# spawner1145/vae-tagger

Measured on AMD Instinct MI355X. Metric: images/sec encode+tag, 1024^2 bf16, higher is better.
Workload: dtype bf16

## Files before the change

### include/vae_tagger_hip.h

```cpp
#ifndef VAE_TAGGER_HIP_H
#define VAE_TAGGER_HIP_H

#include <stddef.h>
#include <stdint.h>

#ifdef __cplusplus
extern "C" {
#endif

typedef struct vt_context vt_context;

enum { VT_OK = 0, VT_ERR_INVALID = 1, VT_ERR_HIP = 2, VT_ERR_STATE = 3, VT_ERR_MISSING_WEIGHT = 4,
       VT_ERR_WORKSPACE = 5 };
enum { VT_F32 = 0, VT_BF16 = 1, VT_F16 = 2, VT_U8 = 3  };

const char* vt_version(void);
int vt_create(int device, vt_context** out);
void vt_destroy(vt_context* ctx);
const char* vt_last_error(const vt_context* ctx);

int vt_encoder_configure(vt_context* ctx, int in_channels, int latent_channels, const int* block_out_channels,
                         int n_blocks, int layers_per_block, int norm_num_groups, float scaling_factor,
                         int has_scaling_factor, float shift_factor, int has_shift_factor);
int vt_set_weight(vt_context* ctx, const char* name, const void* host_data, int dtype, const int64_t* shape,
// ... 107 lines not shown
                    size_t workspace_bytes, void* stream);
int vt_head_forward_backward(vt_context* ctx, void* state, size_t state_bytes, const float* features, const void* labels, int labels_dtype,
                             int B, int loss_kind, double focal_alpha, double focal_gamma, const float* class_weights, double loss_scale,
                             int train, const float* dropout_p , unsigned long long seed, unsigned long long step,
                             float* logits_out, unsigned char* masks_out, void* workspace, size_t workspace_bytes, void* stream);
int vt_head_clip(vt_context* ctx, void* state, size_t state_bytes, float max_norm, void* stream);
int vt_head_step(vt_context* ctx, void* state, size_t state_bytes, double lr, double beta1, double beta2, double eps, double weight_decay,
                 long long t, void* stream);
int vt_head_commit(vt_context* ctx, const void* state, size_t state_bytes, void* stream);
int vt_head_read(vt_context* ctx, const void* state, size_t state_bytes, int kind, const char* name, void* out, size_t out_bytes, void* stream);
int vt_head_write(vt_context* ctx, void* state, size_t state_bytes, int kind, const char* name, const void* src, size_t src_bytes,
                  void* stream);

int vt_set_flag(vt_context* ctx, int flag, int value);

int vt_debug_trace(vt_context* ctx, int enable, unsigned long long* sums_out, int max_sums, int* n_out);
int vt_profile_num_configs(void);
int vt_profile_begin(vt_context* ctx);
int vt_profile_end(vt_context* ctx, int max_cfg, long long* launches, double* total_ms, double* total_flops,
                   const char** kernel_names);

int vt_op_conv2d(vt_context* ctx, const void* x_bf16_nhwc, const void* w_bf16_ohwi, const float* bias,
                 const float* residual_f32, float* out_f32, void* out_bf16, int B, int Hin, int Win, int Cin,
                 int Cout, int ksize, int stride, int pad_lo, int pad_hi, void* stream);
int vt_op_norm_silu_conv3x3(vt_context* ctx, const void* x_nhwc, int x_dtype, const float* scale_shift,
                            const void* w_bf16_ohwi, const float* bias, const float* residual_f32, float* out_f32,
                            void* out_bf16, int B, int H, int W, int Cin, int Cout, void* stream);
size_t vt_op_conv2d_gn_workspace_bytes(int B, int Hout, int Wout, int Cout);
int vt_op_conv2d_gn(vt_context* ctx, const void* x_bf16_nhwc, const void* w_bf16_ohwi, const float* bias,
                    const float* residual_f32, float* out_f32, void* out_bf16, int B, int Hin, int Win, int Cin,
// ... 25 lines not shown
```

### vae_tagger_amd/_lib.py

```python
import ctypes
import os
import threading

_HERE = os.path.dirname(os.path.abspath(__file__))
LIB_PATH = os.environ.get("VAE_TAGGER_HIP_LIB") or os.path.join(_HERE, "csrc", "libvae_tagger_hip.so")

VT_F32, VT_BF16, VT_F16, VT_U8 = 0, 1, 2, 3
VT_STATUS_NONFINITE, VT_STATUS_FP8_SATURATED = 1, 2
ENCODE_MOMENTS, ENCODE_MODE, ENCODE_MODE_SCALED = 0, 1, 2
HEAD_PARAM, HEAD_GRAD, HEAD_ADAM_M, HEAD_ADAM_V, HEAD_LOSS_RING, HEAD_NORM = range(6)
HEAD_LOSS_KINDS = {"bce": 0, "focal": 1, "class_balanced": 2}
HEAD_RING = 256
VT_SAMPLE_GT, VT_SAMPLE_GE = 0, 1

_c = ctypes
_vp, _i, _f, _sz, _ll = _c.c_void_p, _c.c_int, _c.c_float, _c.c_size_t, _c.c_longlong


class ResizeItem(_c.Structure):
    _fields_ = [("src_hwc", _vp), ("src_h", _i), ("src_w", _i), ("crop_left", _i), ("crop_top", _i), ("crop_w", _i), ("crop_h", _i)]


class EvalSource(_c.Structure):
    _fields_ = [("state", _vp), ("state_bytes", _sz), ("capacity", _ll), ("n_seen", _ll)]
# ... 56 lines not shown
    "vt_decoder_feature_dim": (_i, [_vp]),
    "vt_decode_features": (_i, [_vp, _vp, _i, _i, _i, _vp, _vp, _sz, _vp]),
    "vt_head_state_bytes": (_sz, [_vp]),
    "vt_head_workspace_bytes": (_sz, [_vp, _i]),
    "vt_head_init": (_i, [_vp, _vp, _sz, _vp]),
    "vt_head_forward": (_i, [_vp, _vp, _sz, _vp, _i, _vp, _vp, _sz, _vp]),
    "vt_head_forward_backward": (_i, [_vp, _vp, _sz, _vp, _vp, _i, _i, _i, _c.c_double, _c.c_double, _vp, _c.c_double, _i,
                                      _c.POINTER(_f), _c.c_ulonglong, _c.c_ulonglong, _vp, _vp, _vp, _sz, _vp]),
    "vt_head_clip": (_i, [_vp, _vp, _sz, _f, _vp]),
    "vt_head_step": (_i, [_vp, _vp, _sz, _c.c_double, _c.c_double, _c.c_double, _c.c_double, _c.c_double, _ll, _vp]),
    "vt_head_commit": (_i, [_vp, _vp, _sz, _vp]),
    "vt_head_read": (_i, [_vp, _vp, _sz, _i, _c.c_char_p, _vp, _sz, _vp]),
    "vt_head_write": (_i, [_vp, _vp, _sz, _i, _c.c_char_p, _vp, _sz, _vp]),
    "vt_encoder_flops": (_c.c_double, [_vp, _i, _i]),
    "vt_set_flag": (_i, [_vp, _i, _i]),
    "vt_debug_trace": (_i, [_vp, _i, _c.POINTER(_c.c_ulonglong), _i, _c.POINTER(_i)]),
    "vt_profile_num_configs": (_i, []),
    "vt_profile_begin": (_i, [_vp]),
    "vt_profile_end": (_i, [_vp, _i, _c.POINTER(_ll), _c.POINTER(_c.c_double), _c.POINTER(_c.c_double), _c.POINTER(_c.c_char_p)]),
    "vt_op_conv2d": (_i, [_vp, _vp, _vp, _vp, _vp, _vp, _vp, _i, _i, _i, _i, _i, _i, _i, _i, _i, _vp]),
    "vt_op_norm_silu_conv3x3": (_i, [_vp, _vp, _i, _vp, _vp, _vp, _vp, _vp, _vp, _i, _i, _i, _i, _i, _vp]),
    "vt_op_conv2d_gn_workspace_bytes": (_sz, [_i, _i, _i, _i]),
    "vt_op_conv2d_gn": (_i, [_vp, _vp, _vp, _vp, _vp, _vp, _vp, _i, _i, _i, _i, _i, _i, _i, _i, _i, _i, _f, _vp, _vp, _vp, _vp, _vp]),
    "vt_op_conv3x3_fp8_workspace_bytes": (_sz, [_i, _i, _i, _i, _i]),
    "vt_op_conv3x3_fp8": (_i, [_vp, _vp, _vp, _vp, _vp, _vp, _i, _i, _i, _i, _i, _i, _vp, _vp]),
    "vt_op_gemm_nt": (_i, [_vp, _vp, _vp, _vp, _vp, _vp, _i, _i, _i, _i, _i, _i, _i, _ll, _ll, _ll, _f, _i, _vp]),
    "vt_op_conv_in": (_i, [_vp, _vp, _vp, _vp, _vp, _vp, _i, _i, _i, _i, _vp, _vp]),
    "vt_op_groupnorm_workspace_bytes": (_sz, [_i, _i, _i]),
    "vt_op_groupnorm": (_i, [_vp, _vp, _i, _i, _i, _i, _i, _f, _vp, _vp, _i, _vp, _vp, _vp]),
    "vt_op_softmax_rows": (_i, [_vp, _vp, _vp, _i, _i, _i, _i, _vp]),
# ... 81 lines not shown
```

### vae_tagger_amd/csrc/attention.hip

```cpp
#include <math.h>

#include "vt_context.h"

namespace vt {
namespace {

size_t attn_pitch(int S) {
    const size_t ld = (size_t)(S + 7) / 8 * 8;
    return (ld * 2) % 2048 == 0 ? ld + 2048 + 64 : ld;
}
size_t attn_pitch8(int S) {
    const size_t ld = (size_t)(S + 15) / 16 * 16;
    return ld % 2048 == 0 ? ld + 2048 + 64 : ld;
}
constexpr float FP8_QK_SCALE = 8.0f;
constexpr float FP8_P_SCALE_LOG2 = 8.0f;
constexpr float FP8_P_SCALE_SAMPLED_LOG2 = 5.0f;
int attn_group(int B, int S) {
    const size_t ld = attn_pitch(S);
    const size_t per_img = (size_t)S * ld * 4;
    size_t g = ((size_t)37 << 28) / (per_img ? per_img : 1);
    if (g < 1) g = 1;
    if (g > (size_t)B) g = (size_t)B;
    const size_t ngroups = ((size_t)B + g - 1) / g;
// ... 46 lines not shown
bool attn_proj_is_fp8(const vt_context* c, const AttnW& w, int S, int C) { return attn_is_fp8(c, S, C) && c->proj_fp8 && w.wqk8 && w.wv8; }

namespace {

int split_for(long long qblocks, int nkt) { int n = 1; while (n < nkt && qblocks * n < 512) n *= 2; return n < nkt ? n : nkt; }
int sweep_nsplit(int qblocks, int ktiles, int min_tiles) { int n = qblocks > 128 ? 1 : qblocks > 64 ? 2 : 4; while (n > 1 && ktiles / n < min_tiles) n >>= 1; return n; }

struct AttnRun {
    vt_context* c; const AttnW& w; const AttnScratch& sc; int B, S, C; hipStream_t s;
    int ld;
    int lp;
    int ld8, kext8;
    bool f8, p8;
    float scale;
    int mode;
    bool qk_kernel() const { return c->attn_qk_kernel && vt_attn_qk_supported(S, C); }
    ConvGemmArgs gemm() const {
        ConvGemmArgs a{};
        a.zeros = c->zeros; a.ksize = 1; a.stride = 1; a.pad = 0; a.Hin = a.Hout = 1; a.alpha = 1.f;
        return a;
    }
};

int attn_project(const AttnRun& r, const bf16_t* x16, bool x_e4m3) {
    vt_context* c = r.c; const AttnW& w = r.w; const AttnScratch& sc = r.sc; hipStream_t s = r.s;
    const int B = r.B, S = r.S, C = r.C, lp = r.lp;
    if (r.p8) {
        const unsigned char* x8 = (const unsigned char*)x16;
        if (!x_e4m3) {
            std::vector<float> id((size_t)B * C * 2);
// ... 16 lines not shown
        pv.out8 = sc.vt8; pv.ldo = r.ld8; pv.o_bs = (long long)C * r.ld8; pv.kext = r.kext8;
        pv.qbias = w.bv; pv.alpha = w.sv / FP8_ACT_SCALE; pv.oscale = FP8_QK_SCALE; pv.status = c->status;
        pv.C = C; pv.batch = B; pv.zeros = c->zeros;
        pv.nsplit = split_for((long long)B * ((C + 255) / 256), (S + 127) / 128);
        VTCK(profiled(c, s, VT_PROF_PROJ_FP8, 2.0 * B * (double)S * 2 * C * C, "attn qk proj fp8", [&] { return vt_launch_proj_fp8(pq, s); }));
        return profiled(c, s, VT_PROF_PROJ_FP8, 2.0 * B * (double)S * C * C, "attn v proj fp8", [&] { return vt_launch_proj_fp8(pv, s); });
    }
    if (c->attn_proj_kernel && r.qk_kernel() && (lp % 8) == 0) {
        AttnQkArgs pq{};
        pq.mode = 4; pq.q = x16; pq.ldq = C; pq.qk_bs = (long long)S * C; pq.S = S; pq.C = C;
        pq.k = w.wqk; pq.ldk = C; pq.k_bs = 0; pq.nk = 2 * C; pq.kbias = w.bqk;
        pq.P = sc.qk; pq.ldp = 2 * C; pq.p_bs = (long long)S * 2 * C; pq.alpha = 1.f; pq.batch = B; pq.zeros = c->zeros; pq.row_bs = S;
        pq.nsplit = split_for((long long)B * ((S + 255) / 256), (2 * C + 63) / 64);
        AttnQkArgs pv{};
        pv.mode = 4; pv.q = w.wv; pv.ldq = C; pv.qk_bs = 0; pv.S = C; pv.C = C; pv.qbias = w.bv;
        pv.k = x16; pv.ldk = C; pv.k_bs = (long long)S * C; pv.nk = S;
        pv.P = sc.vt; pv.ldp = lp; pv.p_bs = (long long)C * lp; pv.alpha = 1.f; pv.batch = B; pv.zeros = c->zeros; pv.row_bs = C;
        pv.nsplit = split_for((long long)B * ((C + 255) / 256), (S + 63) / 64);
        VTCK(profiled(c, s, VT_PROF_PROJ_BF16, 2.0 * B * (double)S * 2 * C * C, "attn qk proj", [&] { return vt_launch_attn_qk(pq, s); }));
        return profiled(c, s, VT_PROF_PROJ_BF16, 2.0 * B * (double)S * C * C, "attn v proj", [&] { return vt_launch_attn_qk(pv, s); });
    }
    ConvGemmArgs a = r.gemm();
    a.X = x16; a.W = w.wqk; a.bias = w.bqk; a.bias_mode = 1; a.out_bf16 = sc.qk;
    a.Win = a.Wout = S; a.Cin = C; a.Cout = 2 * C; a.Wrows = 2 * C; a.ldx = C; a.ldw = C; a.ldo = 2 * C;
    a.x_bs = (long long)S * C; a.w_bs = 0; a.o_bs = (long long)S * 2 * C; a.batch = B;
    VTCK(launch_gemm(c, a, s, "attn qk proj"));
    a.X = w.wv; a.W = x16; a.bias = w.bv; a.bias_mode = 2; a.out_bf16 = sc.vt;
    a.Win = a.Wout = C; a.Cin = C; a.Cout = r.ld; a.Wrows = S; a.ldx = C; a.ldw = C; a.ldo = lp;
    a.x_bs = 0; a.w_bs = (long long)S * C; a.o_bs = (long long)C * lp; a.batch = B;
    return launch_gemm(c, a, s, "attn v proj");
}

int attn_group_fp8(const AttnRun& r, int b0, int nb) {
    vt_context* c = r.c; const AttnScratch& sc = r.sc; hipStream_t s = r.s;
    const int S = r.S, C = r.C;
// ... 77 lines not shown
    HIPCK(c, vt_launch_attn_qk(k, s), "attn row max");
    k.mode = 2; k.P = sc.probs; k.ldp = lp; k.p_bs = (long long)S * lp; k.rowin = shift; k.rowout = rinv; k.gate = nullptr;
    const bool frag_pv = c->attn_pv_kernel && vt_attn_pv_supported(S, C);
    if (frag_pv) {
        if ((size_t)4 * nb * S > sc.group * attn_slots_bound(S) * (size_t)S) return c->fail(VT_ERR_WORKSPACE, "attention: segment sums exceed the scratch");
        k.p_frag = 1; k.p_bs = vt_attn_pt_elems(S);
        k.rowout = sc.part; k.split_stride = (long long)nb * S;
        k.nsplit = sweep_nsplit(nb * ((S + 255) / 256), (S + 63) / 64, 8);
    }
    VTCK(profiled(c, s, VT_PROF_ATTN_QK, 2.0 * nb * (double)S * S * C, "attn exp scores", [&] { return vt_launch_attn_qk(k, s); }));
    if (!frag_pv) return attn_pv_gemm(r, a, b0, rinv);
    AttnPvArgs v{};
    v.Pt = sc.probs; v.pt_bs = vt_attn_pt_elems(S); v.vt = sc.vt + (long long)b0 * C * lp; v.ldv = lp; v.vt_bs = (long long)C * lp;
    v.rsum = sc.part; v.split_stride = (long long)nb * S; v.row_bs = S; v.o = sc.o + (long long)b0 * S * C; v.ldo = C; v.o_bs = (long long)S * C;
    v.S = S; v.C = C; v.batch = nb; v.zeros = c->zeros;
    return profiled(c, s, VT_PROF_ATTN_PV, 2.0 * nb * (double)S * S * C, "attn pv", [&] { return vt_launch_attn_pv(v, s); });
}

int attn_out_proj(const AttnRun& r, const void* res, void* out, GnState* gn, int groups, int rdt) {
    vt_context* c = r.c; const AttnW& w = r.w; const AttnScratch& sc = r.sc; hipStream_t s = r.s;
    const int B = r.B, S = r.S, C = r.C;
    if (gn) gn->parts = 0;
    if (c->attn_proj_kernel && r.qk_kernel() && (C % 16) == 0) {
        AttnQkArgs po{};
        po.mode = 5; po.q = sc.o; po.ldq = C; po.qk_bs = (long long)S * C; po.S = S; po.C = C;
        po.k = w.wo; po.ldk = C; po.k_bs = 0; po.nk = C; po.kbias = w.bo;
        po.ldp = C; po.p_bs = (long long)S * C; po.alpha = 1.f; po.batch = B; po.zeros = c->zeros; po.row_bs = S;
        if (rdt == 1) { po.res_f32 = (const float*)res; po.out_f32 = (float*)out; } else { po.res_f16 = (const f16_t*)res; po.out_f16 = (f16_t*)out; }
        if (gn && c->fuse_gn_stats && C / groups == 16) { po.gn_partial = gn->partial; po.gn_parts = vt_attn_linear_parts(S); gn->parts = po.gn_parts; }
        po.nsplit = split_for((long long)B * ((S + 255) / 256), (C + 63) / 64);
// ... 5 lines not shown
    a.Win = a.Wout = S; a.Cin = C; a.Cout = C; a.Wrows = C; a.ldx = C; a.ldw = C; a.ldo = C; a.ldr = C;
    a.x_bs = (long long)S * C; a.w_bs = 0; a.o_bs = a.x_bs; a.r_bs = a.x_bs; a.batch = B;
    const int cpg = C / groups;
    if (gn && c->fuse_gn_stats && (cpg == 4 || cpg == 8 || cpg == 16) && C > 32 && (C % (C <= 128 ? 128 : 256)) == 0) {
        a.short_tiles = c->gemm_short;
        a.gn_partial = gn->partial; a.gn_cpg = cpg; gn->parts = vt_conv_gemm_ptiles_of(a);
    }
    return launch_gemm(c, a, s, "attn out proj");
}

}

int run_attention(vt_context* c, const AttnW& w, const bf16_t* x16, const void* res, void* out, int B, int S,
                  const AttnScratch& sc, hipStream_t s, GnState* gn, int groups, int rdt, bool x_e4m3) {
    const int C = w.c;
    const AttnRun r{c, w, sc, B, S, C, s, (S + 7) / 8 * 8, (int)attn_pitch(S), (int)attn_pitch8(S), (S + 15) / 16 * 16,
                    attn_is_fp8(c, S, C), attn_proj_is_fp8(c, w, S, C), 1.0f / sqrtf((float)C), c->attn_mode};
    if (x_e4m3 && !r.p8) return c->fail(VT_ERR_STATE, "internal: e4m3 tokens for a bf16 projection");
    VTCK(attn_project(r, x16, x_e4m3));
    if (r.f8) {
        HIPCK(c, hipMemsetAsync(sc.flags, 0, (size_t)((B + sc.group - 1) / sc.group) * 4, s), "attn flags");
        if (!r.p8) HIPCK(c, vt_launch_attn_row_norms_fp8(sc.qk, (long long)B * S, C, FP8_QK_SCALE, sc.qk8, sc.qn, sc.kn, sc.sd, c->status, s), "attn q|k -> e4m3");
    } else if (r.mode == 0) {
        HIPCK(c, hipMemsetAsync(sc.flags, 0, (size_t)((B + sc.group - 1) / sc.group) * 4, s), "attn flags");
        HIPCK(c, vt_launch_attn_row_norms(sc.qk, (long long)B * S, C, sc.qn, sc.kn, sc.sd, s), "attn row norms");
        HIPCK(c, vt_launch_attn_shift(sc.qn, sc.kn, sc.sd, B, S, r.scale, 120.f, sc.shift, sc.flags, sc.group, s), "attn shift");
    }
    if (r.f8 && !r.p8) HIPCK(c, vt_launch_attn_vt_to_fp8(sc.vt, (long long)C * r.lp, r.lp, sc.vt8, (long long)C * r.ld8, r.ld8, S, r.kext8, C, B, FP8_QK_SCALE, c->status, s), "attn v^T fp8");
    for (int b0 = 0; b0 < B; b0 += sc.group) VTCK(attn_group_scores_pv(r, b0, B - b0 < sc.group ? B - b0 : sc.group));
    return attn_out_proj(r, res, out, gn, groups, rdt);
}

}

using namespace vt;

extern "C" {

size_t vt_op_attention_workspace_bytes(int B, int S, int C) {
    if (B <= 0 || S <= 0 || C <= 0) return 0;
    return attn_scratch_bytes(B, S, C) + ALIGN;
}

int vt_op_attention(vt_context* c, const void* x16, const float* res, float* out, int B, int S, int C, void* ws, void* stream) {
// ... 10 lines not shown
```

### vae_tagger_amd/csrc/attn_pv.hip

```cpp
#include <hip/hip_runtime.h>

#include "vt_common.h"
#include "vt_kernels.h"

namespace {

constexpr int QB = 256;
constexpr int KT = 64;
constexpr int DCH = 512;
constexpr int ROWB = KT * 2;

template <int CB>
__global__ __launch_bounds__(512, 2) void attn_pv_kernel(const AttnPvArgs a) {
    constexpr int VBUF = CB * ROWB;
    constexpr int NCT = CB / 16;
    constexpr int NCP = DCH / CB;
    extern __shared__ __attribute__((aligned(16))) char smem[];
    const int lane = threadIdx.x & 63;
    const int wave = __builtin_amdgcn_readfirstlane(threadIdx.x >> 6);
    const int fr = lane & 15, fq = lane >> 4;
    const int qblocks = (a.S + QB - 1) / QB;
    const int logical = vt_xcd_remap(blockIdx.x, gridDim.x);
    const int cb = logical % NCP;
    const int rest = logical / NCP;
    const int b = rest / qblocks, qb = rest - b * qblocks;
    const int nkt = (a.S + KT - 1) / KT;
    const int nslab = (a.S + 31) / 32;
    const int slab = qb * 8 + wave;
// ... 51 lines not shown
        for (int idx = 0; idx < 2 * NCT; ++idx) {
            if (idx + AHEAD < 2 * NCT) af[(idx + AHEAD) & 7] = frag(idx + AHEAD);
            const int h = idx / NCT, ct = idx % NCT;
#pragma unroll
            for (int j = 0; j < 2; ++j)
                acc[ct][j] = __builtin_amdgcn_mfma_f32_16x16x32_bf16(af[idx & 7], pf[j][h], acc[ct][j], 0, 0, 0);
            __builtin_amdgcn_sched_barrier(0);
        }
        if (kt + 1 < nkt) {
#pragma unroll
            for (int j = 0; j < 2; ++j)
#pragma unroll
                for (int h = 0; h < 2; ++h) pf[j][h] = pn[j][h];
        }
    }
    if (!slab_real) return;
#pragma unroll
    for (int j = 0; j < 2; ++j) {
        const int row = slab * 32 + j * 16 + fr;
        if (row >= a.S) continue;
        const float* ps = a.rsum + (long long)b * a.row_bs + row;
        const float rs = 1.f / (((ps[0] + ps[a.split_stride]) + ps[2 * a.split_stride]) + ps[3 * a.split_stride]);
        bf16_t* o = a.o + (long long)b * a.o_bs + (long long)row * a.ldo + cb * CB + 16 * fq;
#pragma unroll
        for (int G = 0; G < CB / 64; ++G)
#pragma unroll
            for (int i = 0; i < 4; i += 2) {
                bf16x8 hv;
#pragma unroll
                for (int r = 0; r < 4; ++r) { hv[r] = (bf16_t)(acc[4 * G + i][j][r] * rs); hv[4 + r] = (bf16_t)(acc[4 * G + i + 1][j][r] * rs); }
                *(bf16x8*)(o + 64 * G + 4 * i) = hv;
            }
    }
}

}

bool vt_attn_pv_supported(int S, int C) { return C == DCH && S > 0; }
long long vt_attn_pt_elems(int S) { return (long long)((S + 31) / 32) * vt_attn_pt_slab_stride(S); }

hipError_t vt_launch_attn_pv(const AttnPvArgs& a, hipStream_t s) {
    if (!a.Pt || !a.vt || !a.rsum || !a.o || !a.zeros || a.batch <= 0 || !vt_attn_pv_supported(a.S, a.C)) return hipErrorInvalidValue;
    if ((a.ldv % 8) || (a.vt_bs % 8) || (a.ldo % 8) || (a.o_bs % 8) || (a.pt_bs % 8) || a.row_bs < a.S) return hipErrorInvalidValue;
    if (a.ldv < (a.S + 7) / 8 * 8 || (long long)a.C * a.ldv >= (1LL << 31)) return hipErrorInvalidValue;
    if (a.split_stride < (long long)a.batch * a.row_bs) return hipErrorInvalidValue;
    const long long qblk = (long long)((a.S + QB - 1) / QB) * a.batch;
    const bool narrow = qblk * 2 < 192;
    const long long nblk = qblk * (narrow ? 4 : 2);
    if (nblk > 0x7fffffffLL) return hipErrorInvalidValue;
    static std::atomic<unsigned long long> attr_done{0};
    hipError_t ea = vt_once_per_device(attr_done, [&] {
        hipError_t e = hipFuncSetAttribute((const void*)attn_pv_kernel<256>, hipFuncAttributeMaxDynamicSharedMemorySize, 2 * 256 * ROWB);
        if (e == hipSuccess) e = hipFuncSetAttribute((const void*)attn_pv_kernel<128>, hipFuncAttributeMaxDynamicSharedMemorySize, 2 * 128 * ROWB);
        return e;
    });
    if (ea != hipSuccess) return ea;
    if (narrow) hipLaunchKernelGGL(attn_pv_kernel<128>, dim3((unsigned)nblk), dim3(512), 2 * 128 * ROWB, s, a);
// ... 4 lines not shown
```

### vae_tagger_amd/csrc/capi.hip

```cpp
#include <math.h>
#include <string.h>

#include "vt_context.h"
#include "vt_eval.h"

using namespace vt;

namespace {
__global__ void dbg_checksum_kernel(const unsigned int* __restrict__ p, long long n, unsigned long long* __restrict__ out) {
    unsigned long long acc = 0;
    for (long long i = (long long)blockIdx.x * blockDim.x + threadIdx.x; i < n; i += (long long)gridDim.x * blockDim.x) acc += (unsigned long long)p[i] * (unsigned long long)(i % 1021 + 1);
    atomicAdd(out, acc);
}
constexpr int DBG_SLOTS = 256;
}

void vt::dbg_sum(vt_context* c, const void* p, size_t bytes, hipStream_t s) {
    if (!c->dbg_on || !c->dbg || c->dbg_n >= DBG_SLOTS) return;
    hipLaunchKernelGGL(dbg_checksum_kernel, dim3(64), dim3(256), 0, s, (const unsigned int*)p, (long long)(bytes / 4), c->dbg + c->dbg_n);
    ++c->dbg_n;
}

extern "C" {

// ... 426 lines not shown
    if (flag == 3) { c->halo_occ2 = value < 0 ? 0 : (value > 4 ? 4 : value); return VT_OK; }
    if (flag == 4) { c->res_fp16 = value != 0; return VT_OK; }
    if (flag == 5) { c->conv_in_mfma = value != 0; return VT_OK; }
    if (flag == 6) { c->gemm_short = value != 0; return VT_OK; }
    if (flag == 8) { c->fuse_shortcut = value != 0; return VT_OK; }
    if (flag == 9) { c->attn_qk_kernel = value != 0; return VT_OK; }
    if (flag == 10) { c->pv_stream = value != 0; return VT_OK; }
    if (flag == 11) { c->fp8 = value != 0; return VT_OK; }
    if (flag == 16) { if ((value & 3) == 3 || value < 0 || value > 7) return c->fail(VT_ERR_INVALID, "vt_set_flag(16): tile shape 0..2 (+4: every layer)"); c->fp8_tile = value; return VT_OK; }
    if (flag == 12) { c->attn_pv_kernel = value != 0; return VT_OK; }
    if (flag == 17) { c->attn_proj_kernel = value != 0; return VT_OK; }
    if (flag == 18) { c->f16_ops = value != 0; return VT_OK; }
    if (flag == 19) { c->s2_planar = value != 0; return VT_OK; }
    if (flag == 21) { c->eval_merge_vec = value != 0; return VT_OK; }
    if (flag == 20) { c->conv_out_halo = value != 0; return VT_OK; }
    if (flag == 13) { c->s2_halo = value != 0; return VT_OK; }
    if (flag == 14) { c->attn_fp8 = value != 0; return VT_OK; }
    if (flag == 15) { c->proj_fp8 = value != 0; return VT_OK; }
    if (flag == 7) {
        if (value < 0 || value > 2) return c->fail(VT_ERR_INVALID, "vt_set_flag(7): value %d not in 0..2", value);
        c->attn_mode = value;
        return VT_OK;
    }
    return c->fail(VT_ERR_INVALID, "vt_set_flag: unknown flag %d", flag);
}

int vt_profile_num_configs(void) { return VT_NUM_PROF_SLOTS; }

int vt_preprocess_u8(vt_context* c, const uint8_t* in_hwc, int B, int H, int W, float* out_nchw, void* stream) {
    if (!c) return VT_ERR_INVALID;
// ... 157 lines not shown
```

### vae_tagger_amd/csrc/vt_context.h

```cpp
#pragma once
#include <hip/hip_runtime.h>
#include <stdarg.h>
#include <stdio.h>

#include <array>
#include <map>
#include <string>
#include <vector>

#include "../../include/vae_tagger_hip.h"
#include "vt_decoder.h"
#include "vt_kernels.h"

namespace vt {

struct HostTensor {
    std::vector<float> v;
    std::vector<int64_t> shape;
    int64_t numel() const { int64_t n = 1; for (auto d : shape) n *= d; return n; }
};

struct ConvW {
    const bf16_t* w = nullptr; const bf16_t* wp = nullptr; const float* b = nullptr; int cin = 0, cout = 0, k = 0;
    const bf16_t* wp2 = nullptr;
    const bf16_t* wpo = nullptr; const bf16_t* wpo16 = nullptr;
    const bf16_t* w16 = nullptr; const bf16_t* wp16 = nullptr; const bf16_t* wp2_16 = nullptr;
    const unsigned char* wp8 = nullptr; const float* mult8 = nullptr;
    const unsigned char* w8g = nullptr; const float* mult8g = nullptr;
    const unsigned char* wp8s2 = nullptr;
};
struct NormW { const float* g = nullptr; const float* b = nullptr; int c = 0; };
struct ResnetW {
    NormW n1, n2; ConvW c1, c2, sc; bool has_sc = false; int cin = 0, cout = 0;
    const bf16_t* sc_wp = nullptr; const float* b_c2sc = nullptr;
    const bf16_t* sc_wp16 = nullptr;
    const bf16_t* sc_wp8 = nullptr;
};
struct AttnW { NormW gn; const bf16_t *wqk = nullptr, *wv = nullptr, *wo = nullptr; const float *bqk = nullptr, *bv = nullptr, *bo = nullptr; int c = 0;
               const unsigned char *wqk8 = nullptr, *wv8 = nullptr; float sqk = 1.f, sv = 1.f; };
struct StageW { std::vector<ResnetW> res; bool has_down = false; ConvW down; };

struct EncoderW {
    bool configured = false, finalized = false;
    int in_ch = 3, latent = 16, layers = 2, groups = 32;
    std::vector<int> block_out;
    float scaling = 1.f, shift = 0.f;
    bool has_scaling = false, has_shift = false;
    const bf16_t* conv_in_wpk = nullptr;
    const float* conv_in_w = nullptr;
    const float* conv_in_b = nullptr;
    std::vector<StageW> stages;
    ResnetW mid0, mid1;
    AttnW attn;
    NormW norm_out;
// ... 27 lines not shown
    int fuse_shortcut = 1;
    int pv_stream = 1;
    int attn_qk_kernel = 1;
    int attn_pv_kernel = 1;
    int fp8 = 0;
    int halo_occ2 = 3;
    int gemm_short = 1;
    int proj_fp8 = 1;
    int attn_fp8 = 1;
    unsigned long long* dbg = nullptr; int dbg_n = 0; bool dbg_on = false;
    int conv_out_halo = 1;
    int s2_planar = 1;
    int eval_merge_vec = 1;
    int f16_ops = 0;
    int attn_proj_kernel = 1;
    int fp8_tile = 0;
    int s2_halo = 1;
    int* rs_host = nullptr; size_t rs_host_ints = 0; hipEvent_t rs_event = nullptr;
    struct RsRingSlot { void* host = nullptr; size_t bytes = 0; hipEvent_t ev = nullptr; bool used = false; };
    static constexpr int RS_RING = 4;
    RsRingSlot rs_ring[RS_RING];
    unsigned rs_ring_next = 0;
    std::map<std::array<int, 4>, std::vector<int>> rs_tables;
    int conv_in_mfma = 1;
    void* op_scratch = nullptr; size_t op_scratch_bytes = 0;

    struct ProfRec { hipEvent_t e0, e1; double flops; int cfg; };
    bool profiling = false;
    std::vector<ProfRec> prof;
    std::vector<hipEvent_t> event_pool;
// ... 58 lines not shown
    HIPCK(c, hipEventRecord(r.e1, s), "hipEventRecord");
    c->prof.push_back(r);
    return VT_OK;
}

float bf2f(uint16_t h);
float h2f(uint16_t h);
std::vector<float> pack_conv_in(const float* w_o27, int cout);
std::vector<uint16_t> pack_conv_in_mfma(const float* w_o27, const float* bias);
struct ConvE4m3 {
    std::vector<uint8_t> wp8;  std::vector<float> mult8;
    std::vector<uint8_t> w8g;  std::vector<float> mult8g;
    std::vector<uint8_t> wp8s2;
};
ConvE4m3 pack_conv_e4m3(const float* w_oihw, int cout, int cin, bool s2_layout);

int rs_ksize(int in_size, int out_size, int kind);
void rs_table(int in_size, int out_size, int kind, int* tab);

void dbg_sum(vt_context* c, const void* p, size_t bytes, hipStream_t s);

struct GnState {
    float* partial = nullptr; float* ss = nullptr;
    int parts = 0;
};
struct ScFuse { const bf16_t* x; const bf16_t* wp; const float* bias; int cin; const bf16_t* wp8; const bf16_t* wp16;
                bool x_f16;
};
struct ConvOpts {
    GnState* gn = nullptr;
// ... 30 lines not shown
```

### vae_tagger_amd/csrc/vt_kernels.h

```cpp
#pragma once
#include <hip/hip_runtime.h>
#include "vt_common.h"

struct ConvGemmArgs {
    const bf16_t* X;
    const bf16_t* W;
    const float* bias;
    const float* res;
    const f16_t* res_f16;
    float* out_f32;
    bf16_t* out_bf16;
    f16_t* out_f16;
    const void* zeros;
    float* gn_partial;
    int Hin, Win, Hout, Wout;
    int Cin, Cout;
    int Wrows;
    int ksize, stride, pad;
    int ldx, ldw, ldo, ldr;
    long long x_bs, w_bs, o_bs, r_bs;
    int batch;
    float alpha;
    int bias_mode;
    int out_mode;
// ... 49 lines not shown
    int nk, ldk; long long k_bs; const float* kbias; const float* qbias;
    const f16_t* res_f16; const float* res_f32; f16_t* out_f16; float* out_f32; float* gn_partial; int gn_parts;
};
int vt_attn_linear_parts(int S);
bool vt_attn_qk_supported(int S, int C);
hipError_t vt_launch_attn_qk(const AttnQkArgs& a, hipStream_t s);

struct AttnPvArgs {
    const bf16_t* Pt; long long pt_bs;
    const bf16_t* vt; int ldv; long long vt_bs;
    const float* rsum; long long row_bs;
    long long split_stride;
    bf16_t* o; int ldo; long long o_bs;
    int S, C, batch;
    const void* zeros;
};
bool vt_attn_pv_supported(int S, int C);
__host__ __device__ inline long long vt_attn_pt_slab_stride(int S) { return (long long)((S + 63) / 64) * 2048 + 1152; }
long long vt_attn_pt_elems(int S);
hipError_t vt_launch_attn_pv(const AttnPvArgs& a, hipStream_t s);

struct AttnQk8Args {
    const unsigned char* qk8; int ldq; long long qk_bs;
    int S, C;
    unsigned char* P8; long long p_bs;
    const float* rowin;
    float* rowout;
    long long row_bs;
    float alpha;
    float pscale_log2;
// ... 183 lines not shown
```

### vae_tagger_amd/csrc/weights.hip

```cpp
#include <math.h>
#include <string.h>

#include "vt_context.h"

namespace vt {

static uint16_t f2bf(float f) {
    uint32_t u;
    memcpy(&u, &f, 4);
    if ((u & 0x7fffffffu) > 0x7f800000u) return (uint16_t)((u >> 16) | 0x40);
    u += 0x7fffu + ((u >> 16) & 1u);
    return (uint16_t)(u >> 16);
}
float bf2f(uint16_t h) { uint32_t u = (uint32_t)h << 16; float f; memcpy(&f, &u, 4); return f; }
static uint16_t f2h(float f) { const _Float16 h = (_Float16)f; uint16_t u; memcpy(&u, &h, 2); return u; }
float h2f(uint16_t h) {
    const uint32_t s = (h >> 15) & 1, e = (h >> 10) & 31, m = h & 1023;
    uint32_t u;
    if (e == 0) {
        if (m == 0) u = s << 31;
        else { int sh = 0; uint32_t mm = m; while (!(mm & 1024)) { mm <<= 1; ++sh; } u = (s << 31) | ((uint32_t)(113 - sh) << 23) | ((mm & 1023) << 13); }
    } else if (e == 31) u = (s << 31) | 0x7f800000u | (m << 13);
    else u = (s << 31) | ((e + 112) << 23) | (m << 13);
    float f; memcpy(&f, &u, 4); return f;
// ... 163 lines not shown
    }
    return pk;
}

static int get_conv_in(vt_context* c, EncoderW& e) {
    const int c0 = e.block_out[0];
    const HostTensor* w = c->find("encoder.conv_in.weight");
    const HostTensor* b = c->find("encoder.conv_in.bias");
    if (!w || !b) return c->fail(VT_ERR_MISSING_WEIGHT, "missing weight encoder.conv_in.{weight,bias}");
    if (w->numel() != (int64_t)c0 * 27 || b->numel() != c0) return c->fail(VT_ERR_INVALID, "shape mismatch for encoder.conv_in");
    if (!up(c, &e.conv_in_w, pack_conv_in(w->v.data(), c0)) || !up(c, &e.conv_in_b, b->v)) return c->fail(VT_ERR_HIP, "upload failed for conv_in");
    if (c0 == 128 && e.groups == 32 && !up(c, &e.conv_in_wpk, pack_conv_in_mfma(w->v.data(), b->v.data()))) return c->fail(VT_ERR_HIP, "upload failed for conv_in");
    return VT_OK;
}

static int get_attention(vt_context* c, const std::string& a, int C, AttnW* at) {
    VTCK(get_norm(c, a + ".group_norm", C, &at->gn));
    std::vector<uint16_t> wqk, wv, wo; std::vector<float> bqk, bv, bo;
    VTCK(get_linear_bf16(c, a + ".to_q", C, C, &wqk, &bqk));
    VTCK(get_linear_bf16(c, a + ".to_k", C, C, &wqk, &bqk));
    VTCK(get_linear_bf16(c, a + ".to_v", C, C, &wv, &bv));
    VTCK(get_linear_bf16(c, a + ".to_out.0", C, C, &wo, &bo));
    at->c = C;
    auto pack8 = [&](const std::vector<uint16_t>& w, float* scale) {
        std::vector<float> f(w.size());
        for (size_t i = 0; i < w.size(); ++i) f[i] = bf2f(w[i]);
        *scale = e4m3_scale(f.data(), f.size());
        std::vector<uint8_t> o(w.size());
        for (size_t i = 0; i < w.size(); ++i) o[i] = f2e4m3(f[i] / *scale);
        return o;
    };
    const bool ok = up(c, &at->wqk, wqk) && up(c, &at->wv, wv) && up(c, &at->wo, wo) && up(c, &at->bqk, bqk) && up(c, &at->bv, bv) && up(c, &at->bo, bo) &&
                    up(c, &at->wqk8, pack8(wqk, &at->sqk)) && up(c, &at->wv8, pack8(wv, &at->sv));
    return ok ? VT_OK : c->fail(VT_ERR_HIP, "upload failed for attention");
}

}

using namespace vt;

extern "C" int vt_encoder_finalize(vt_context* c) {
    if (!c) return VT_ERR_INVALID;
    EncoderW& e = c->enc;
    if (!e.configured) return c->fail(VT_ERR_STATE, "vt_encoder_configure was not called");
    DeviceGuard guard(c);
    e.finalized = false;
    e.conv_in_wpk = nullptr; e.conv_in_w = nullptr; e.conv_in_b = nullptr;
    e.stages.clear(); e.mid0 = ResnetW(); e.mid1 = ResnetW(); e.attn = AttnW(); e.norm_out = NormW(); e.conv_out = ConvW();
    c->free_allocs(c->enc_allocs);
    c->cur_allocs = &c->enc_allocs;
    VTCK(get_conv_in(c, e));
    int ci = e.block_out[0];
    for (size_t i = 0; i < e.block_out.size(); ++i) {
        StageW st;
// ... 27 lines not shown
```

Baseline: 218.1.

## Fold attention V and output projections into one weight and fuse epilogue into PV

Precomputes Wo·Wv and the combined bias on the host at weight load, so the V projection directly produces output-projected values. The PV kernel then applies the softmax normalisation, folded bias, residual add and optional GroupNorm partial statistics in its epilogue. This removes the separate output-projection GEMM and its intermediate read and write. In exchange, the folded weight is rounded to bf16 after the product, which changes numerics slightly. The epilogue also raises register pressure in the PV kernel.

```diff
diff --git a/include/vae_tagger_hip.h b/include/vae_tagger_hip.h
--- a/include/vae_tagger_hip.h
+++ b/include/vae_tagger_hip.h
@@ -145,6 +145,8 @@
 
 int vt_set_flag(vt_context* ctx, int flag, int value);
 
+int vt_fold_attention_weights(const float* wv, const float* wo, const float* bv, const float* bo, int C, uint16_t* wov_bf16, float* bov);
+
 int vt_debug_trace(vt_context* ctx, int enable, unsigned long long* sums_out, int max_sums, int* n_out);
 int vt_profile_num_configs(void);
 int vt_profile_begin(vt_context* ctx);
diff --git a/vae_tagger_amd/_lib.py b/vae_tagger_amd/_lib.py
--- a/vae_tagger_amd/_lib.py
+++ b/vae_tagger_amd/_lib.py
@@ -94,6 +94,7 @@
     "vt_head_write": (_i, [_vp, _vp, _sz, _i, _c.c_char_p, _vp, _sz, _vp]),
     "vt_encoder_flops": (_c.c_double, [_vp, _i, _i]),
     "vt_set_flag": (_i, [_vp, _i, _i]),
+    "vt_fold_attention_weights": (_i, [_vp, _vp, _vp, _vp, _i, _vp, _vp]),
     "vt_debug_trace": (_i, [_vp, _i, _c.POINTER(_c.c_ulonglong), _i, _c.POINTER(_i)]),
     "vt_profile_num_configs": (_i, []),
     "vt_profile_begin": (_i, [_vp]),
diff --git a/vae_tagger_amd/csrc/attention.hip b/vae_tagger_amd/csrc/attention.hip
--- a/vae_tagger_amd/csrc/attention.hip
+++ b/vae_tagger_amd/csrc/attention.hip
@@ -84,6 +84,8 @@
     bool f8, p8;
     float scale;
     int mode;
+    bool fold_o;
+    const void* res; void* out; GnState* gn; int rdt;
     bool qk_kernel() const { return c->attn_qk_kernel && vt_attn_qk_supported(S, C); }
     ConvGemmArgs gemm() const {
         ConvGemmArgs a{};
@@ -130,11 +132,12 @@
         pq.nsplit = split_for((long long)B * ((S + 255) / 256), (2 * C + 63) / 64);
         AttnQkArgs pv{};
         pv.mode = 4; pv.q = w.wv; pv.ldq = C; pv.qk_bs = 0; pv.S = C; pv.C = C; pv.qbias = w.bv;
+        if (r.fold_o) { pv.q = w.wov; pv.qbias = nullptr; }
         pv.k = x16; pv.ldk = C; pv.k_bs = (long long)S * C; pv.nk = S;
         pv.P = sc.vt; pv.ldp = lp; pv.p_bs = (long long)C * lp; pv.alpha = 1.f; pv.batch = B; pv.zeros = c->zeros; pv.row_bs = C;
         pv.nsplit = split_for((long long)B * ((C + 255) / 256), (S + 63) / 64);
         VTCK(profiled(c, s, VT_PROF_PROJ_BF16, 2.0 * B * (double)S * 2 * C * C, "attn qk proj", [&] { return vt_launch_attn_qk(pq, s); }));
-        return profiled(c, s, VT_PROF_PROJ_BF16, 2.0 * B * (double)S * C * C, "attn v proj", [&] { return vt_launch_attn_qk(pv, s); });
+        return profiled(c, s, VT_PROF_PROJ_BF16, (r.fold_o ? 4.0 : 2.0) * B * (double)S * C * C, "attn v proj", [&] { return vt_launch_attn_qk(pv, s); });
     }
     ConvGemmArgs a = r.gemm();
     a.X = x16; a.W = w.wqk; a.bias = w.bqk; a.bias_mode = 1; a.out_bf16 = sc.qk;
@@ -242,6 +245,13 @@
     v.Pt = sc.probs; v.pt_bs = vt_attn_pt_elems(S); v.vt = sc.vt + (long long)b0 * C * lp; v.ldv = lp; v.vt_bs = (long long)C * lp;
     v.rsum = sc.part; v.split_stride = (long long)nb * S; v.row_bs = S; v.o = sc.o + (long long)b0 * S * C; v.ldo = C; v.o_bs = (long long)S * C;
     v.S = S; v.C = C; v.batch = nb; v.zeros = c->zeros;
+    if (r.fold_o) {
+        const long long e0 = (long long)b0 * S * C;
+        v.o = nullptr; v.bias = r.w.bov;
+        if (r.rdt == 1) { v.res_f32 = r.res ? (const float*)r.res + e0 : nullptr; v.out_f32 = (float*)r.out + e0; }
+        else { v.res_f16 = r.res ? (const f16_t*)r.res + e0 : nullptr; v.out_f16 = (f16_t*)r.out + e0; }
+        if (r.gn && r.gn->parts) { v.gn_parts = r.gn->parts; v.gn_partial = r.gn->partial + (long long)b0 * r.gn->parts * (C / 16) * 3; }
+    }
     return profiled(c, s, VT_PROF_ATTN_PV, 2.0 * nb * (double)S * S * C, "attn pv", [&] { return vt_launch_attn_pv(v, s); });
 }
 
@@ -277,8 +287,11 @@
 int run_attention(vt_context* c, const AttnW& w, const bf16_t* x16, const void* res, void* out, int B, int S,
                   const AttnScratch& sc, hipStream_t s, GnState* gn, int groups, int rdt, bool x_e4m3) {
     const int C = w.c;
-    const AttnRun r{c, w, sc, B, S, C, s, (S + 7) / 8 * 8, (int)attn_pitch(S), (int)attn_pitch8(S), (S + 15) / 16 * 16,
-                    attn_is_fp8(c, S, C), attn_proj_is_fp8(c, w, S, C), 1.0f / sqrtf((float)C), c->attn_mode};
+    AttnRun r{c, w, sc, B, S, C, s, (S + 7) / 8 * 8, (int)attn_pitch(S), (int)attn_pitch8(S), (S + 15) / 16 * 16,
+              attn_is_fp8(c, S, C), attn_proj_is_fp8(c, w, S, C), 1.0f / sqrtf((float)C), c->attn_mode};
+    r.fold_o = c->attn_fold && !c->fp8 && r.mode != 2 && c->attn_proj_kernel && r.qk_kernel() && (r.lp % 8) == 0 && c->attn_pv_kernel &&
+               vt_attn_pv_supported(S, C) && w.wov && w.bov && (C % 16) == 0;
+    r.res = res; r.out = out; r.gn = gn; r.rdt = rdt;
     if (x_e4m3 && !r.p8) return c->fail(VT_ERR_STATE, "internal: e4m3 tokens for a bf16 projection");
     VTCK(attn_project(r, x16, x_e4m3));
     if (r.f8) {
@@ -290,7 +303,9 @@
         HIPCK(c, vt_launch_attn_shift(sc.qn, sc.kn, sc.sd, B, S, r.scale, 120.f, sc.shift, sc.flags, sc.group, s), "attn shift");
     }
     if (r.f8 && !r.p8) HIPCK(c, vt_launch_attn_vt_to_fp8(sc.vt, (long long)C * r.lp, r.lp, sc.vt8, (long long)C * r.ld8, r.ld8, S, r.kext8, C, B, FP8_QK_SCALE, c->status, s), "attn v^T fp8");
+    if (r.fold_o && gn) gn->parts = (c->fuse_gn_stats && C / groups == 16) ? vt_attn_linear_parts(S) : 0;
     for (int b0 = 0; b0 < B; b0 += sc.group) VTCK(attn_group_scores_pv(r, b0, B - b0 < sc.group ? B - b0 : sc.group));
+    if (r.fold_o) return VT_OK;
     return attn_out_proj(r, res, out, gn, groups, rdt);
 }
 
diff --git a/vae_tagger_amd/csrc/attn_pv.hip b/vae_tagger_amd/csrc/attn_pv.hip
--- a/vae_tagger_amd/csrc/attn_pv.hip
+++ b/vae_tagger_amd/csrc/attn_pv.hip
@@ -11,7 +11,7 @@
 constexpr int ROWB = KT * 2;
 
 template <int CB>
-__global__ __launch_bounds__(512, 2) void attn_pv_kernel(const AttnPvArgs a) {
+__global__ __launch_bounds__(512, 2) VT_NO_PACKED_F32 void attn_pv_kernel(const AttnPvArgs a) {
     constexpr int VBUF = CB * ROWB;
     constexpr int NCT = CB / 16;
     constexpr int NCP = DCH / CB;
@@ -93,6 +93,93 @@
                 for (int h = 0; h < 2; ++h) pf[j][h] = pn[j][h];
         }
     }
+    if (a.out_f16 || a.out_f32) {
+        typedef _Float16 f16x8 __attribute__((ext_vector_type(8)));
+        const int ngroups = DCH / 16;
+        float* gp = a.gn_partial ? a.gn_partial + (((long long)b * a.gn_parts + slab) * ngroups + (cb * CB) / 16 + fq) * 3 : nullptr;
+        if (!slab_real) {
+            if (gp && fr == 0) {
+#pragma unroll
+                for (int G = 0; G < CB / 64; ++G) { gp[12 * G] = 0.f; gp[12 * G + 1] = 0.f; gp[12 * G + 2] = 0.f; }
+            }
+            return;
+        }
+        const int nrows = a.S - slab * 32 > 32 ? 32 : a.S - slab * 32;
+        float rs[2]; bool ok[2]; long long off[2];
+#pragma unroll
+        for (int j = 0; j < 2; ++j) {
+            const int row = slab * 32 + j * 16 + fr;
+            ok[j] = row < a.S;
+            rs[j] = 0.f;
+            if (ok[j]) {
+                const float* ps = a.rsum + (long long)b * a.row_bs + row;
+                rs[j] = 1.f / (((ps[0] + ps[a.split_stride]) + ps[2 * a.split_stride]) + ps[3 * a.split_stride]);
+            }
+            off[j] = (long long)b * a.o_bs + (long long)row * a.ldo + cb * CB + 16 * fq;
+        }
+#pragma unroll
+        for (int G = 0; G < CB / 64; ++G) {
+            float bias[16];
+#pragma unroll
+            for (int i = 0; i < 4; ++i) {
+                const f32x4 bv = *(const f32x4*)(a.bias + cb * CB + 64 * G + 16 * fq + 4 * i);
+#pragma unroll
+                for (int r = 0; r < 4; ++r) bias[4 * i + r] = bv[r];
+            }
+            float v[2][16];
+#pragma unroll
+            for (int j = 0; j < 2; ++j) {
+                float res[16];
+#pragma unroll
+                for (int e = 0; e < 16; ++e) res[e] = 0.f;
+                const long long o = off[j] + 64 * G;
+                if (ok[j] && a.res_f16) {
+                    const f16x8 r0 = *(const f16x8*)(a.res_f16 + o), r1 = *(const f16x8*)(a.res_f16 + o + 8);
+#pragma unroll
+                    for (int e = 0; e < 8; ++e) { res[e] = (float)r0[e]; res[8 + e] = (float)r1[e]; }
+                } else if (ok[j] && a.res_f32) {
+#pragma unroll
+                    for (int i = 0; i < 4; ++i) {
+                        const f32x4 r4 = *(const f32x4*)(a.res_f32 + o + 4 * i);
+#pragma unroll
+                        for (int r = 0; r < 4; ++r) res[4 * i + r] = r4[r];
+                    }
+                }
+#pragma unroll
+                for (int i = 0; i < 4; ++i)
+#pragma unroll
+                    for (int r = 0; r < 4; ++r) v[j][4 * i + r] = fmaf(acc[4 * G + i][j][r], rs[j], bias[4 * i + r]) + res[4 * i + r];
+                if (ok[j] && a.out_f16) {
+                    f16x8 h0, h1;
+#pragma unroll
+                    for (int e = 0; e < 8; ++e) { h0[e] = (f16_t)v[j][e]; h1[e] = (f16_t)v[j][8 + e]; }
+                    *(f16x8*)(a.out_f16 + o) = h0;
+                    *(f16x8*)(a.out_f16 + o + 8) = h1;
+                } else if (ok[j]) {
+#pragma unroll
+                    for (int i = 0; i < 4; ++i) *(f32x4*)(a.out_f32 + o + 4 * i) = f32x4{v[j][4 * i], v[j][4 * i + 1], v[j][4 * i + 2], v[j][4 * i + 3]};
+                }
+            }
+            if (gp) {
+                const float piv = __shfl(v[0][0], lane & 48, 64);
+                float s1 = 0.f, s2 = 0.f;
+#pragma unroll
+                for (int j = 0; j < 2; ++j) {
+                    if (ok[j]) {
+#pragma unroll
+                        for (int e = 0; e < 16; ++e) { const float d = v[j][e] - piv; s1 += d; s2 = fmaf(d, d, s2); }
+                    }
+                }
+                s1 = vt_row16_sum(s1); s2 = vt_row16_sum(s2);
+                if (fr == 0) {
+                    const float n = (float)nrows * 16.f;
+                    const float ms = s1 / n;
+                    gp[12 * G] = n; gp[12 * G + 1] = piv + ms; gp[12 * G + 2] = fmaxf(s2 - s1 * ms, 0.f);
+                }
+            }
+        }
+        return;
+    }
     if (!slab_real) return;
 #pragma unroll
     for (int j = 0; j < 2; ++j) {
@@ -119,7 +206,10 @@
 long long vt_attn_pt_elems(int S) { return (long long)((S + 31) / 32) * vt_attn_pt_slab_stride(S); }
 
 hipError_t vt_launch_attn_pv(const AttnPvArgs& a, hipStream_t s) {
-    if (!a.Pt || !a.vt || !a.rsum || !a.o || !a.zeros || a.batch <= 0 || !vt_attn_pv_supported(a.S, a.C)) return hipErrorInvalidValue;
+    const bool folded = a.out_f16 || a.out_f32;
+    if (!a.Pt || !a.vt || !a.rsum || (!a.o && !folded) || !a.zeros || a.batch <= 0 || !vt_attn_pv_supported(a.S, a.C)) return hipErrorInvalidValue;
+    if (folded && ((a.out_f16 && a.out_f32) || (a.res_f16 && a.res_f32) || !a.bias || (a.ldo % 16) || (a.o_bs % 16) || a.ldo < a.C)) return hipErrorInvalidValue;
+    if (folded && a.gn_partial && a.gn_parts != vt_attn_linear_parts(a.S)) return hipErrorInvalidValue;
     if ((a.ldv % 8) || (a.vt_bs % 8) || (a.ldo % 8) || (a.o_bs % 8) || (a.pt_bs % 8) || a.row_bs < a.S) return hipErrorInvalidValue;
     if (a.ldv < (a.S + 7) / 8 * 8 || (long long)a.C * a.ldv >= (1LL << 31)) return hipErrorInvalidValue;
     if (a.split_stride < (long long)a.batch * a.row_bs) return hipErrorInvalidValue;
diff --git a/vae_tagger_amd/csrc/capi.hip b/vae_tagger_amd/csrc/capi.hip
--- a/vae_tagger_amd/csrc/capi.hip
+++ b/vae_tagger_amd/csrc/capi.hip
@@ -464,6 +464,7 @@
     if (flag == 19) { c->s2_planar = value != 0; return VT_OK; }
     if (flag == 21) { c->eval_merge_vec = value != 0; return VT_OK; }
     if (flag == 20) { c->conv_out_halo = value != 0; return VT_OK; }
+    if (flag == 22) { c->attn_fold = value != 0; return VT_OK; }
     if (flag == 13) { c->s2_halo = value != 0; return VT_OK; }
     if (flag == 14) { c->attn_fp8 = value != 0; return VT_OK; }
     if (flag == 15) { c->proj_fp8 = value != 0; return VT_OK; }
diff --git a/vae_tagger_amd/csrc/vt_context.h b/vae_tagger_amd/csrc/vt_context.h
--- a/vae_tagger_amd/csrc/vt_context.h
+++ b/vae_tagger_amd/csrc/vt_context.h
@@ -37,7 +37,8 @@
     const bf16_t* sc_wp8 = nullptr;
 };
 struct AttnW { NormW gn; const bf16_t *wqk = nullptr, *wv = nullptr, *wo = nullptr; const float *bqk = nullptr, *bv = nullptr, *bo = nullptr; int c = 0;
-               const unsigned char *wqk8 = nullptr, *wv8 = nullptr; float sqk = 1.f, sv = 1.f; };
+               const unsigned char *wqk8 = nullptr, *wv8 = nullptr; float sqk = 1.f, sv = 1.f;
+               const bf16_t* wov = nullptr; const float* bov = nullptr; };
 struct StageW { std::vector<ResnetW> res; bool has_down = false; ConvW down; };
 
 struct EncoderW {
@@ -95,6 +96,7 @@
     int eval_merge_vec = 1;
     int f16_ops = 0;
     int attn_proj_kernel = 1;
+    int attn_fold = 1;
     int fp8_tile = 0;
     int s2_halo = 1;
     int* rs_host = nullptr; size_t rs_host_ints = 0; hipEvent_t rs_event = nullptr;
@@ -183,6 +185,7 @@
     std::vector<uint8_t> wp8s2;
 };
 ConvE4m3 pack_conv_e4m3(const float* w_oihw, int cout, int cin, bool s2_layout);
+void fold_attention_weights(const float* wv, const float* wo, const float* bv, const float* bo, int C, uint16_t* wov, float* bov);
 
 int rs_ksize(int in_size, int out_size, int kind);
 void rs_table(int in_size, int out_size, int kind, int* tab);
diff --git a/vae_tagger_amd/csrc/vt_kernels.h b/vae_tagger_amd/csrc/vt_kernels.h
--- a/vae_tagger_amd/csrc/vt_kernels.h
+++ b/vae_tagger_amd/csrc/vt_kernels.h
@@ -87,6 +87,8 @@
     bf16_t* o; int ldo; long long o_bs;
     int S, C, batch;
     const void* zeros;
+    const float* bias; const f16_t* res_f16; const float* res_f32; f16_t* out_f16; float* out_f32;
+    float* gn_partial; int gn_parts;
 };
 bool vt_attn_pv_supported(int S, int C);
 __host__ __device__ inline long long vt_attn_pt_slab_stride(int S) { return (long long)((S + 63) / 64) * 2048 + 1152; }
diff --git a/vae_tagger_amd/csrc/weights.hip b/vae_tagger_amd/csrc/weights.hip
--- a/vae_tagger_amd/csrc/weights.hip
+++ b/vae_tagger_amd/csrc/weights.hip
@@ -201,6 +201,22 @@
     return VT_OK;
 }
 
+void fold_attention_weights(const float* wv, const float* wo, const float* bv, const float* bo, int C, uint16_t* wov, float* bov) {
+    std::vector<double> acc((size_t)C * C, 0.0);
+    for (int i = 0; i < C; ++i) {
+        double* row = acc.data() + (size_t)i * C;
+        double b = 0.0;
+        for (int o = 0; o < C; ++o) {
+            const double a = wo[(size_t)i * C + o];
+            const float* src = wv + (size_t)o * C;
+            for (int k = 0; k < C; ++k) row[k] += a * (double)src[k];
+            b += a * (double)bv[o];
+        }
+        bov[i] = (float)(b + (double)bo[i]);
+    }
+    for (size_t i = 0; i < acc.size(); ++i) wov[i] = f2bf((float)acc[i]);
+}
+
 static int get_attention(vt_context* c, const std::string& a, int C, AttnW* at) {
     VTCK(get_norm(c, a + ".group_norm", C, &at->gn));
     std::vector<uint16_t> wqk, wv, wo; std::vector<float> bqk, bv, bo;
@@ -217,14 +233,24 @@
         for (size_t i = 0; i < w.size(); ++i) o[i] = f2e4m3(f[i] / *scale);
         return o;
     };
+    std::vector<uint16_t> wov((size_t)C * C); std::vector<float> bov(C);
+    fold_attention_weights(c->find(a + ".to_v.weight")->v.data(), c->find(a + ".to_out.0.weight")->v.data(), c->find(a + ".to_v.bias")->v.data(),
+                           c->find(a + ".to_out.0.bias")->v.data(), C, wov.data(), bov.data());
     const bool ok = up(c, &at->wqk, wqk) && up(c, &at->wv, wv) && up(c, &at->wo, wo) && up(c, &at->bqk, bqk) && up(c, &at->bv, bv) && up(c, &at->bo, bo) &&
-                    up(c, &at->wqk8, pack8(wqk, &at->sqk)) && up(c, &at->wv8, pack8(wv, &at->sv));
+                    up(c, &at->wqk8, pack8(wqk, &at->sqk)) && up(c, &at->wv8, pack8(wv, &at->sv)) &&
+                    up(c, &at->wov, wov) && up(c, &at->bov, bov);
     return ok ? VT_OK : c->fail(VT_ERR_HIP, "upload failed for attention");
 }
 
 }
 
 using namespace vt;
+
+extern "C" int vt_fold_attention_weights(const float* wv, const float* wo, const float* bv, const float* bo, int C, uint16_t* wov_bf16, float* bov) {
+    if (!wv || !wo || !bv || !bo || !wov_bf16 || !bov || C <= 0) return VT_ERR_INVALID;
+    fold_attention_weights(wv, wo, bv, bo, C, wov_bf16, bov);
+    return VT_OK;
+}
 
 extern "C" int vt_encoder_finalize(vt_context* c) {
     if (!c) return VT_ERR_INVALID;
```

New measurement: 218.6, median of 6. Within noise of the previous version (+0.2%).
